# wangjiarui153/AIGV-Assessor

Measured on AMD Instinct MI355X. Metric: scored clips/sec (8-frame 448x448, InternVL2-8B stage-2 score eval), higher is better.
Workload: dtype bf16

## Files before the change

### aigv-assessor_amd/csrc/context.hip

```cpp
#include <cstdarg>
#include <cstdio>
#include <cstring>
#include <new>

#include "ctx.h"

using namespace aigv;

static thread_local std::string g_err;

int aigv::fail(aigv_ctx* c, int code, const char* fmt, ...) {
  char buf[512];
  va_list ap;
  va_start(ap, fmt);
  vsnprintf(buf, sizeof buf, fmt, ap);
  va_end(ap);
  if (c) c->err = buf;
  g_err = buf;
  return code;
}

static_assert(AIGV_MAX_KV_CAPACITY == AIGV_DECODE_MAX_CHUNKS * AIGV_DECODE_KEYS_PER_CHUNK, "the header's bound is the decode merge pass's");

static const char* kv_capacity_check(int kv_capacity) {
// ... 71 lines not shown
    if ((rc = dalloc(c, &c->l_t, T * k.llm_hidden))) break;
    if ((rc = dalloc(c, &c->l_qkv, T * c->qkv_out))) break;
    if ((rc = dalloc(c, &c->l_ao, T * k.llm_hidden))) break;
    if ((rc = dalloc(c, &c->l_ffn, T * k.llm_inter))) break;
    if ((rc = dalloc(c, &c->l_rows, (size_t)(k.max_out_rows + k.max_seqs + 64) * k.llm_hidden))) break;
    if ((rc = dalloc(c, &c->l_pos, T))) break;
    if ((rc = dalloc(c, &c->l_seq, T))) break;
    if ((rc = dalloc(c, &c->l_cu, (size_t)k.max_seqs + 1))) break;
    if ((rc = dalloc(c, &c->l_rowidx, (size_t)k.max_out_rows + k.max_seqs + 64))) break;
    if ((rc = dalloc(c, &c->l_rowidx2, (size_t)k.max_out_rows + k.max_seqs + 64))) break;
    if ((rc = dalloc(c, &c->l_kvlen, (size_t)k.max_seqs))) break;
    if ((rc = dalloc(c, &c->l_packed, (size_t)64))) break;
    if ((rc = dalloc(c, &c->l_trim, (size_t)64 * (2 * k.llm_hidden + k.llm_inter)))) break;
    if ((rc = dalloc(c, &c->l_trim_h, (size_t)(k.max_out_rows + k.max_seqs + 64) * k.llm_hidden))) break;
    if ((rc = dalloc(c, &c->l_neg1, (size_t)k.max_tokens))) break;
    c->rp_vit = RowPlan(); c->rp_llm = RowPlan(); c->cur_rp = nullptr;
    c->rp_vit.cap_halves = (int)(vr / 128) + 2 * k.vit_chunk + 2;
    c->rp_llm.cap_halves = (int)(T / 128) + 2 * k.max_seqs + 2;
    if ((rc = dalloc(c, &c->rp_vit.d_tab, (size_t)2 * c->rp_vit.cap_halves))) break;
    if ((rc = dalloc(c, &c->rp_llm.d_tab, (size_t)2 * c->rp_llm.cap_halves))) break;
    {
      const size_t widest = (size_t)std::max(std::max(std::max(2 * k.llm_inter, c->qkv_out), std::max(k.vit_inter, 3 * k.vit_hidden)), k.llm_hidden);
      const size_t rows = std::max((size_t)k.max_tokens, (size_t)k.vit_chunk * c->S);
      c->splitk_floats = std::min(SPLITK_MAX_FLOATS, (size_t)8 * rows * widest);
      void* p = nullptr;
      if (hipMalloc(&p, c->splitk_floats * sizeof(float)) != hipSuccess) { rc = fail(c, AIGV_ERR_ALLOC, "hipMalloc(split-K scratch) failed"); break; }
      c->ws_allocs.push_back(p);
      c->splitk_ws = (float*)p;
      if (hipMalloc(&p, c->splitk_floats * sizeof(float)) != hipSuccess) { rc = fail(c, AIGV_ERR_ALLOC, "hipMalloc(split-K scratch, InternViT) failed"); break; }
      c->ws_allocs.push_back(p);
      c->splitk_ws_vit = (float*)p;
    }
    if (hipMemset(c->l_neg1, 0xFF, (size_t)k.max_tokens * sizeof(int32_t)) != hipSuccess) { rc = fail(c, AIGV_ERR_HIP, "hipMemset failed"); break; }
    {
      int maxd = k.llm_hidden;
// ... 341 lines not shown
```

### aigv-assessor_amd/csrc/ctx.h

```cpp
#pragma once
#include <hip/hip_runtime.h>

#include <algorithm>
#include <string>
#include <unordered_map>
#include <vector>

#include "../../include/aigv_amd.h"
#include "kernels.h"

namespace aigv {

struct DevBuf {
  void* p = nullptr;
  size_t bytes = 0;
};

struct VitLayer {
  const bf16_t *ls1, *ls2, *qkv_w, *qkv_b, *qn, *kn, *proj_w, *proj_b, *fc1_w, *fc1_b, *fc2_w, *fc2_b, *n1w, *n1b, *n2w, *n2b;
};
struct LlmLayer {
  const bf16_t *wqkv, *wo, *w13, *w2, *an, *fn;
};

// ... 1 lines not shown
  uint8_t *wqkv = nullptr, *wo = nullptr, *w13 = nullptr, *w2 = nullptr;
  float *s_wqkv = nullptr, *s_wo = nullptr, *s_w13 = nullptr, *s_w2 = nullptr;
};

struct ProfRec {
  int cls;
  hipEvent_t a, b;
  double flops, bytes;
};

struct RowPlan {
  struct Tiny { int row0, stride_rows, count; };
  std::vector<Tiny> tiny;
  int rows = 0, body_halves = 0, tail_halves = 0, tail_rows = 0;
  int32_t* d_tab = nullptr;
  int cap_halves = 0;
};

}

struct aigv_ctx {
  aigv_config cfg{};
  int device = 0;
  std::string err;
  std::unordered_map<std::string, aigv::DevBuf> w;
  std::vector<void*> allocs;
  std::vector<void*> ws_allocs;
  bool ws_phase = false;
  bool finalized = false;
  int np = 0, S = 0, Kp = 0, grid = 0, ntok = 0, proj_in = 0, qkv_out = 0, head_dim = 0, vit_head_dim = 0, g = 0;
// ... 5 lines not shown
               *p_b1[2] = {nullptr, nullptr}, *p_w2[2] = {nullptr, nullptr}, *p_b2[2] = {nullptr, nullptr};
  ScoreHeadArgs score{};
  bf16_t *v_col = nullptr, *v_x = nullptr, *v_t = nullptr, *v_qkv = nullptr, *v_ao = nullptr, *v_h = nullptr;
  int32_t* v_cu = nullptr;
  bf16_t *p_t = nullptr, *p_mid = nullptr;
  bf16_t *l_h = nullptr, *l_t = nullptr, *l_qkv = nullptr, *l_ao = nullptr, *l_ffn = nullptr, *l_rows = nullptr;
  int32_t *l_pos = nullptr, *l_seq = nullptr, *l_cu = nullptr, *l_rowidx = nullptr, *l_rowidx2 = nullptr, *l_kvlen = nullptr;
  unsigned long long* l_packed = nullptr;
  int32_t* l_neg1 = nullptr;
  bool fp8_llm = false;
  bool llm_lin_dirty = false;
  std::vector<aigv::LlmLayerFp8> llm8;
  uint8_t* q8 = nullptr;
  float* q8_scale = nullptr;
  aigv::RowPlan rp_vit, rp_llm;
  const aigv::RowPlan* cur_rp = nullptr;
  bool trim_last_layer = true;
  int attn_round_scores = AIGV_ATTENTION_NUMERICS_DEFAULT;
  int tune[AIGV_TUNE_COUNT];
  aigv_ctx() { std::fill(tune, tune + AIGV_TUNE_COUNT, -1); }
  size_t splitk_floats = 0;
  float* splitk_ws = nullptr;
  float* splitk_ws_vit = nullptr;
  bool on_vit_front = false;
  bf16_t* l_trim = nullptr;
  bf16_t* l_trim_h = nullptr;
  bf16_t* l_score_ws = nullptr;
  bf16_t* l_lp = nullptr;
  int lp_ldo = 0;
  bf16_t *kc = nullptr, *vc = nullptr;
// ... 91 lines not shown

struct Tune {
  int v[AIGV_TUNE_COUNT];
  constexpr int operator[](int knob) const { return v[knob]; }
};
extern Tune g_tune;
inline int tune_knob(const aigv_ctx* c, int knob) { return (c && c->tune[knob] >= 0) ? c->tune[knob] : g_tune.v[knob]; }
inline int resolved_gemm_mode(const aigv_ctx* c) { return tune_knob(c, AIGV_TUNE_GEMM_MODE); }
inline Tune tune_of(const aigv_ctx* c) {
  Tune t;
  for (int k = 0; k < AIGV_TUNE_COUNT; ++k) t.v[k] = tune_knob(c, k);
  return t;
}

GemmArgs gemm_args(const bf16_t* A, int lda, const bf16_t* W, int ldw, bf16_t* C, int ldc, int M, int N, int K);
int build_row_plan(aigv_ctx* c, RowPlan& rp, const int32_t* cu, int n_seq, hipStream_t s);
int launch_one(aigv_ctx* c, const GemmArgs& a, int epi, bool use256, hipStream_t s);
int run_gemm(aigv_ctx* c, const GemmArgs& a, int epi, hipStream_t s);
int run_gemm_rows(aigv_ctx* c, const GemmArgs& a, int epi, const RowPlan& rp, hipStream_t s);
int run_gemm_full(aigv_ctx* c, const GemmArgs& a, int epi, hipStream_t s);
int run_llm_gemm(aigv_ctx* c, const GemmArgs& a, int epi, hipStream_t s);
int run_gemm_fp8(aigv_ctx* c, const bf16_t* A, int lda, int K, const uint8_t* W8, const float* w_scale, bf16_t* C, int ldc, int T, int N,
                 int epi, const bf16_t* resid, int ldr, hipStream_t s);
int run_skinny(aigv_ctx* c, const bf16_t* x, int ldx, int R, const bf16_t* W, int ldw, int N, int K, const bf16_t* bias,
               const bf16_t* resid, int ldr, bf16_t* out, int ldo, int epi, hipStream_t s, int p = 1);
constexpr size_t SPLITK_MAX_FLOATS = (size_t)64 << 20;
int splitk_scratch(aigv_ctx* c, size_t need_floats, float** out);
extern double g_rate256;

}
```

### aigv-assessor_amd/csrc/dispatch.hip

```cpp
#include <mutex>

#include "ctx.h"

namespace aigv {

static GemmArgs tuned(const aigv_ctx* c, const GemmArgs& a) {
  GemmArgs b = a;
  b.order_sel = tune_knob(c, AIGV_TUNE_GEMM256_ORDER); b.variant_sel = tune_knob(c, AIGV_TUNE_GEMM256_VARIANT);
  return b;
}
double g_rate256 = 1.46;
constexpr double KT128 = 0.95, FIX128 = 6.0, LONE128 = 0.70, FIX256 = 9.0, LAUNCH_GAP = 2.0;
static double kt256() { return 2.0 * KT128 / g_rate256; }

static double t256(long row_tiles, int N, int nk) {
  if (row_tiles <= 0) return 0;
  const long tiles = row_tiles * (N / 256);
  return (double)((tiles + 255) / 256) * (nk * kt256() + FIX256);
}
static double t128_blocks(long blocks, double nk_each) {
  const double rt = nk_each * KT128 + FIX128;
  const long full = blocks / 512, part = blocks % 512;
  return full * rt + (part == 0 ? 0.0 : part <= 256 ? LONE128 * rt : rt);
}
// ... 192 lines not shown
      const int sk = skinny_epi(epi);
      ProfScope ps(c, c ? c->gemm_cls : AIGV_PROF_GEMM, 2.0 * bot.M * (double)a.N * a.K, 2.0 * (double)a.N * a.K, s);
      hipError_t e = aigv_launch_skinny_gemm(bot.A, bot.lda, bot.M, bot.W, bot.ldw, bot.N, bot.K, bot.bias, bot.resid, bot.ldr,
                                            bot.C, bot.ldc, sk, s, bot.ls);
      if (e != hipSuccess) return fail(c, AIGV_ERR_HIP, "skinny remainder (M=%d N=%d K=%d): %s", bot.M, bot.N, bot.K, hipGetErrorString(e));
      return 0;
    }
    if (pl.last_slices > 1) return launch_splitk(c, bot, epi, pl.last_slices, false, s);
    return launch_one(c, bot, epi, false, s);
  }
  return 0;
}

constexpr int TINY_TAIL = 4;

int build_row_plan(aigv_ctx* c, RowPlan& rp, const int32_t* cu, int n_seq, hipStream_t s) {
  rp.tiny.clear();
  std::vector<int32_t> body, tail;
  bool uniform = true;
  for (int b = 1; b < n_seq; ++b) uniform = uniform && (cu[b + 1] - cu[b] == cu[1] - cu[0]);
  rp.tail_rows = 0;
  for (int b = 0; b < n_seq; ++b) {
    const int L = cu[b + 1] - cu[b], nb = L / 256, rem = L % 256, r0 = cu[b] + nb * 256;
    for (int j = 0; j < 2 * nb; ++j) { body.push_back(cu[b] + j * 128); body.push_back(128); }
    if (rem == 0) continue;
    if (rem <= TINY_TAIL) {
      if (!uniform) rp.tiny.push_back({r0, 1, rem});
      else if (b == 0)
        for (int j = 0; j < rem; ++j) rp.tiny.push_back({r0 + j, L, n_seq});
      continue;
    }
    tail.push_back(r0); tail.push_back(std::min(rem, 128));
    if (rem > 128) { tail.push_back(r0 + 128); tail.push_back(rem - 128); }
    rp.tail_rows += rem;
  }
  rp.body_halves = (int)body.size() / 2;
  rp.tail_halves = (int)tail.size() / 2;
  rp.rows = cu[n_seq];
  if (rp.body_halves + rp.tail_halves > rp.cap_halves)
    return fail(c, AIGV_ERR_STATE, "row plan: %d half tiles exceed the table's %d", rp.body_halves + rp.tail_halves, rp.cap_halves);
  body.insert(body.end(), tail.begin(), tail.end());
  if (!body.empty()) HIPCHK(c, aigv_launch_write_ints(body.data(), (int)body.size(), rp.d_tab, s));
  return 0;
}

static int tail_slices(int N, int K, int forced) {
  const int tn = N / 256, nk = K / 64;
  int best = 1;
  for (int S : {2, 4, 8})
    if (nk % S == 0 && nk / S >= 8 && 2 * tn * S <= 256) best = S;
  if (forced == 1 || (forced > 1 && nk % forced == 0 && nk / forced >= 4)) best = forced;
  return best;
}

static int launch_tab(aigv_ctx* c, const GemmArgs& a, int epi, const int32_t* tab, int halves, int rows, int S, hipStream_t s) {
  if (halves <= 0) return 0;
  GemmArgs b = tuned(c, a);
// ... 93 lines not shown
    if (!lone) TRY(launch_tab(c, a, epi, rp.d_tab, rp.body_halves, rp.body_halves * 128, 1, s));
  }
  if (tails_apart) {
    const size_t per_pair = (size_t)S * 256 * a.N;
    const size_t cap = c ? c->splitk_floats : SPLITK_MAX_FLOATS;
    const int max_halves = (int)std::min<size_t>(cap / per_pair, 4096) * 2;
    if (max_halves < 2) return fail(c, AIGV_ERR_STATE, "split-K scratch too small for one tail tile (N=%d, %d slices)", a.N, S);
    for (int h0 = 0; h0 < rp.tail_halves; h0 += max_halves) {
      const int nh = std::min(max_halves, rp.tail_halves - h0);
      TRY(launch_tab(c, a, epi, rp.d_tab + 2 * (rp.body_halves + h0), nh, nh * 128, S, s));
    }
  }
  return run_tiny_tails(c, a, epi, rp, s);
}

int run_gemm_full(aigv_ctx* c, const GemmArgs& a, int epi, hipStream_t s) {
  if (const char* m = aigv_gemm_check(a, epi)) return fail(c, AIGV_ERR_ARG, "%s (M=%d N=%d K=%d epi=%d)", m, a.M, a.N, a.K, epi);
  const int mode = resolved_gemm_mode(c);
  if (use_co(c, a, mode)) return launch_co(c, a, epi, s);
  if (mode == 1 || a.N < 256 || (a.N % 256 && epi == EPI_SWIGLU)) return launch_one(c, a, epi, false, s);
  if (a.N % 256) {
    TRY(launch_one(c, col_slice(a, 0, a.N - 128), epi, true, s));
    return launch_one(c, col_slice(a, a.N - 128, 128), epi, false, s);
  }
  return launch_one(c, a, epi, true, s);
}

int run_llm_gemm(aigv_ctx* c, const GemmArgs& a, int epi, hipStream_t s) {
  return c->cur_rp ? run_gemm_rows(c, a, epi, *c->cur_rp, s) : run_gemm(c, a, epi, s);
}
// ... 50 lines not shown
```

### aigv-assessor_amd/csrc/gemm256.hip

```cpp
#include <cstdlib>
#include <type_traits>

#include "common.h"
#include "kernels.h"

namespace {

constexpr int TM = 256, TN = 256, TK = 64;
constexpr int UNIT = 128 * 128;
constexpr int BUF = 4 * UNIT;
constexpr int STAGE_ROWP = 144;
constexpr int STAGE_BYTES = 16 * STAGE_ROWP;
constexpr int LDS_BYTES = 2 * BUF + 8 * STAGE_BYTES;
constexpr int GROUP_M256 = 4;
inline int row_tiles(const GemmArgs& a) { return a.row_tab ? (a.tab_halves + 1) / 2 : (a.M + TM - 1) / TM; }
}
static inline int tile_order(const GemmArgs& a, bool big_w, int nbm) { return a.order_sel > 0 ? a.order_sel - 1 : (big_w && nbm >= 32 ? 4 : 0); }
namespace {

#define RAW_BARRIER() asm volatile("s_barrier" ::: "memory")

#ifdef AIGV_GEMM_STAMP
constexpr int GSTAMP_REPL = 1024;
__device__ unsigned long long g_gemm_stamp[8][2][GSTAMP_REPL][8];
// ... 18 lines not shown
#endif
  (void)policy;
  *(u16x8*)dst = val;
}

template <int EPI, int VAR, bool FP8 = false, bool FUSE = false>
__global__ __launch_bounds__(512, 2) void gemm256_kernel(const GemmArgs p) {
  static_assert(!FP8 || ((VAR & 4) != 0 && EPI != EPI_PATCH), "the fp8 form uses the LDS-staged epilogue (or writes split-K slabs)");
  static_assert(!FUSE || (!FP8 && EPI != EPI_PARTIAL && EPI != EPI_PATCH), "the fused form: bf16, a body epilogue");
  extern __shared__ __attribute__((aligned(16))) char smem[];
  const int tid = threadIdx.x, lane = tid & 63;
  const int wave = __builtin_amdgcn_readfirstlane(tid >> 6);
  const int g = wave >> 2, wc = wave & 3;
  GSTAMP(gs_begin);

  const int nbm = p.row_tab ? (p.tab_halves + 1) / 2 : (p.M + TM - 1) / TM, nbn = p.N / TN;
  const int n_body = nbm * nbn;
  const bool is_slice = FUSE && (int)blockIdx.x >= n_body;
  const int nwg = is_slice ? ((p.fuse_tail_halves + 1) / 2) * nbn * p.k_slices : n_body;
  int wg;
  {
    const int bid = is_slice ? (int)blockIdx.x - n_body : (int)blockIdx.x, xcd = bid & 7, q = nwg >> 3, r = nwg & 7;
    wg = (xcd < r ? xcd * (q + 1) : r * (q + 1) + (xcd - r) * q) + (bid >> 3);
  }
  const bool partial = (EPI == EPI_PARTIAL) || is_slice;
  int slice_idx = (EPI == EPI_PARTIAL) ? (int)blockIdx.y : 0;
  int tm, tn;
  if (is_slice) {
    slice_idx = wg % p.k_slices;
    const int tile = wg / p.k_slices;
    tn = tile % nbn; tm = tile / nbn;
  } else if (p.order == 0) {
    const int per_group = GROUP_M256 * nbn;
    const int grp = wg / per_group, first_m = grp * GROUP_M256;
    const int gsz = min(nbm - first_m, GROUP_M256);
    const int in_g = wg - grp * per_group;
    tm = first_m + in_g % gsz; tn = in_g / gsz;
  } else {
    const int gn = p.order;
    const int per_group = gn * nbm;
    const int grp = wg / per_group, first_n = grp * gn;
    const int gsz = min(nbn - first_n, gn);
    const int in_g = wg - grp * per_group;
    tn = first_n + in_g % gsz; tm = in_g / gsz;
  }
  const int n0 = tn * TN;
  int hb, hv;
  if (p.row_tab) {
    const int h = 2 * tm + g;
    hb = 0; hv = 0;
    if (is_slice) {
      if (h < p.fuse_tail_halves) { hb = p.row_tab[2 * (p.tab_halves + h)]; hv = p.row_tab[2 * (p.tab_halves + h) + 1]; }
    } else if (h < p.tab_halves) { hb = p.row_tab[2 * h]; hv = p.row_tab[2 * h + 1]; }
  } else {
    hb = tm * TM + g * 128; hv = min(p.M - hb, 128);
    if (hv <= 0) { hb = p.M - 1; hv = 0; }
  }
  hb = __builtin_amdgcn_readfirstlane(hb);
  hv = __builtin_amdgcn_readfirstlane(hv);
  const int hend = hb + hv;
  auto relc = [&](int r) { return max(min(r, hv - 1), 0); };
// ... 458 lines not shown
            }
            u16x4 o;
#pragma unroll
            for (int e = 0; e < 4; ++e) o[e] = f2bf(v[e]);
            *(u16x4*)(p.C + orow * p.ldc + n) = o;
          }
      }
    }
  GSTAMP_FINISH();
}

template <int EPI, int VAR>
hipError_t launch256(const GemmArgs& a, hipStream_t s) {
  static LdsAttrOnce lds_attr;
  if (hipError_t e = lds_attr.ensure((const void*)gemm256_kernel<EPI, VAR>, LDS_BYTES); e != hipSuccess) return e;
  const int nbm = row_tiles(a), nbn = a.N / TN;
  GemmArgs b = a;
  b.order = tile_order(a, (size_t)a.N * (size_t)a.K >= ((size_t)32 << 20), nbm);
  hipLaunchKernelGGL((gemm256_kernel<EPI, VAR>), dim3(nbm * nbn), dim3(512), LDS_BYTES, s, b);
  return hipGetLastError();
}

template <int VAR>
hipError_t launch256v(const GemmArgs& a, int epi, hipStream_t s) {
  switch (epi) {
    case EPI_STORE: return launch256<EPI_STORE, VAR>(a, s);
    case EPI_GELU: return launch256<EPI_GELU, VAR>(a, s);
    case EPI_LS_RESID: return launch256<EPI_LS_RESID, VAR>(a, s);
    case EPI_RESID: return launch256<EPI_RESID, VAR>(a, s);
    case EPI_SWIGLU: return launch256<EPI_SWIGLU, VAR>(a, s);
    case EPI_PATCH: return launch256<EPI_PATCH, VAR>(a, s);
// ... 15 lines not shown
          unsigned long long t = 0;
          for (int r = 0; r < GSTAMP_REPL; ++r) t += host[e][c][r][i];
          out[(e * 2 + c) * 8 + i] = t;
        }
  }
  if (reset) {
    for (auto& a : host) for (auto& b : a) for (auto& c : b) for (auto& d : c) d = 0;
    if (hipMemcpyToSymbol(HIP_SYMBOL(g_gemm_stamp), host, sizeof host) != hipSuccess) return -2;
  }
  return 0;
}
#endif


bool aigv_gemm256_supported(const GemmArgs& a) { return a.N % TN == 0 && a.K % TK == 0 && a.M >= 1 && (!a.row_tab || a.tab_halves >= 1); }

template <int EPI>
hipError_t launch256_fp8(const GemmArgs& b, hipStream_t s) {
  static LdsAttrOnce lds_attr;
  if (hipError_t e = lds_attr.ensure((const void*)gemm256_kernel<EPI, 7, true>, LDS_BYTES); e != hipSuccess) return e;
  const int nbm = row_tiles(b), nbn = b.N / TN;
  GemmArgs c = b;
  c.order = tile_order(b, (size_t)b.N * (size_t)b.K * 2 >= ((size_t)64 << 20), nbm);
  hipLaunchKernelGGL((gemm256_kernel<EPI, 7, true>), dim3(nbm * nbn), dim3(512), LDS_BYTES, s, c);
  return hipGetLastError();
}

hipError_t aigv_launch_gemm256_fp8(const GemmArgs& a, int epi, hipStream_t s) {
  if (a.M < 1 || a.N % TN || a.K % 128 || (a.lda % 16) || (a.ldw % 16) || !a.row_scale || !a.col_scale || !a.A || !a.W || !a.C)
    return hipErrorInvalidValue;
  if ((epi == EPI_RESID || epi == EPI_LS_RESID) && (!a.resid || a.ldr % 8)) return hipErrorInvalidValue;
  if (epi == EPI_LS_RESID && !a.ls) return hipErrorInvalidValue;
  if (epi == EPI_SWIGLU && a.bias) return hipErrorInvalidValue;
  GemmArgs b = a;
  b.K = a.K / 2; b.lda = a.lda / 2; b.ldw = a.ldw / 2;
  switch (epi) {
    case EPI_STORE: return launch256_fp8<EPI_STORE>(b, s);
    case EPI_GELU: return launch256_fp8<EPI_GELU>(b, s);
    case EPI_LS_RESID: return launch256_fp8<EPI_LS_RESID>(b, s);
    case EPI_RESID: return launch256_fp8<EPI_RESID>(b, s);
    case EPI_SWIGLU: return launch256_fp8<EPI_SWIGLU>(b, s);
    default: return hipErrorInvalidValue;
  }
}

hipError_t aigv_launch_gemm256_fp8_partial(const GemmArgs& a, hipStream_t s) {
  if (a.M < 1 || a.N % TN || a.K % 128 || (a.lda % 16) || (a.ldw % 16) || !a.row_scale || !a.col_scale || !a.A || !a.W || !a.part || a.k_slices < 1 ||
      (a.K / 128) % a.k_slices)
    return hipErrorInvalidValue;
  static LdsAttrOnce lds_attr;
  if (hipError_t e = lds_attr.ensure((const void*)gemm256_kernel<EPI_PARTIAL, 7, true>, LDS_BYTES); e != hipSuccess) return e;
  GemmArgs b = a;
  b.K = a.K / 2; b.lda = a.lda / 2; b.ldw = a.ldw / 2;
  const int nbm = row_tiles(a), nbn = a.N / TN;
  hipLaunchKernelGGL((gemm256_kernel<EPI_PARTIAL, 7, true>), dim3(nbm * nbn, a.k_slices), dim3(512), LDS_BYTES, s, b);
  return hipGetLastError();
}

hipError_t aigv_launch_gemm256_partial(const GemmArgs& a, hipStream_t s) {
  if (!aigv_gemm256_supported(a) || a.k_slices < 1 || (a.K / TK) % a.k_slices || !a.part) return hipErrorInvalidValue;
  static LdsAttrOnce lds_attr;
  if (hipError_t e = lds_attr.ensure((const void*)gemm256_kernel<EPI_PARTIAL, 7>, LDS_BYTES); e != hipSuccess) return e;
  const int nbm = row_tiles(a), nbn = a.N / TN;
  hipLaunchKernelGGL((gemm256_kernel<EPI_PARTIAL, 7>), dim3(nbm * nbn, a.k_slices), dim3(512), LDS_BYTES, s, a);
  return hipGetLastError();
}

template <int EPI>
static hipError_t launch256_fused(const GemmArgs& a, hipStream_t s) {
  static LdsAttrOnce lds_attr;
  if (hipError_t e = lds_attr.ensure((const void*)gemm256_kernel<EPI, 7, false, true>, LDS_BYTES); e != hipSuccess) return e;
  const int nbm = (a.tab_halves + 1) / 2, nbn = a.N / TN;
  GemmArgs b = a;
  b.order = tile_order(a, (size_t)a.N * (size_t)a.K >= ((size_t)32 << 20), nbm);
  b.fuse_body_wg = nbm * nbn;
  const int grid = nbm * nbn + ((a.fuse_tail_halves + 1) / 2) * nbn * a.k_slices;
  hipLaunchKernelGGL((gemm256_kernel<EPI, 7, false, true>), dim3(grid), dim3(512), LDS_BYTES, s, b);
  return hipGetLastError();
}

hipError_t aigv_launch_gemm256_fused(const GemmArgs& a, int epi, hipStream_t s) {
  if (!aigv_gemm256_supported(a) || !a.row_tab || (a.tab_halves & 1) || a.fuse_tail_halves < 1 || a.k_slices < 2 || (a.K / TK) % a.k_slices || !a.part)
    return hipErrorInvalidValue;
  switch (epi) {
    case EPI_STORE: return launch256_fused<EPI_STORE>(a, s);
    case EPI_GELU: return launch256_fused<EPI_GELU>(a, s);
    case EPI_LS_RESID: return launch256_fused<EPI_LS_RESID>(a, s);
    case EPI_RESID: return launch256_fused<EPI_RESID>(a, s);
    case EPI_SWIGLU: return launch256_fused<EPI_SWIGLU>(a, s);
  }
  return hipErrorInvalidValue;
}

hipError_t aigv_launch_gemm256(const GemmArgs& a, int epi, hipStream_t s) {
  switch (a.variant_sel > 0 ? a.variant_sel - 1 : 1) {
    case 0: return launch256v<0>(a, epi, s);
    case 3: return launch256v<3>(a, epi, s);
    default: return launch256v<7>(a, epi, s);
  }
}
```

### aigv-assessor_amd/csrc/kernels.h

```cpp
#pragma once
#include <hip/hip_runtime.h>
#include <stdint.h>

typedef uint16_t bf16_t;

enum GemmEpilogue {
  EPI_STORE = 0,
  EPI_GELU = 1,
  EPI_LS_RESID = 2,
  EPI_RESID = 3,
  EPI_SWIGLU = 4,
  EPI_PATCH = 5,
  EPI_COUNT = 6,
  EPI_PARTIAL = 6
};

struct GemmArgs {
  const bf16_t* A; int lda;
  const bf16_t* W; int ldw;
  bf16_t* C; int ldc;
  const bf16_t* bias;
  const bf16_t* ls;
  const bf16_t* resid; int ldr;
  const bf16_t* pos;
  int M, N, K;
  int np;
  float* part;
  int k_slices;
  const float* row_scale;
  const float* col_scale;
  const int32_t* row_tab; int tab_halves;
  int fuse_tail_halves, fuse_body_wg;
  int order_sel, variant_sel;
  int order;
};

const char* aigv_gemm_check(const GemmArgs& a, int epi);
hipError_t aigv_launch_gemm(const GemmArgs& a, int epi, hipStream_t s);
hipError_t aigv_launch_gemm_splitk(const GemmArgs& a, int epi, int k_slices, float* ws, hipStream_t s, bool tile256 = false);
hipError_t aigv_launch_gemm256_partial(const GemmArgs& a, hipStream_t s);
hipError_t aigv_launch_gemm256_fp8(const GemmArgs& a, int epi, hipStream_t s);
hipError_t aigv_launch_gemm256_fp8_partial(const GemmArgs& a, hipStream_t s);
hipError_t aigv_launch_gemm_splitk_fp8(const GemmArgs& a, int epi, int k_slices, float* ws, hipStream_t s);
hipError_t aigv_launch_rmsnorm_quant_fp8(const bf16_t* x, int ldx, const bf16_t* w, uint8_t* q, int ldq, float* scale, int rows, int H, float eps,
                                         hipStream_t s);
hipError_t aigv_launch_quant_fp8_rows(const bf16_t* x, int ldx, int rows, int K, uint8_t* q, int ldq, float* scale, hipStream_t s);
bool aigv_gemm256_supported(const GemmArgs& a);
hipError_t aigv_launch_gemm256_fused(const GemmArgs& a, int epi, hipStream_t s);
// ... 122 lines not shown
```

### aigv-assessor_amd/csrc/passes.hip

```cpp
#include <cmath>

#include "ctx.h"

using namespace aigv;

extern "C" {

static int vit_norm(aigv_ctx* c, const bf16_t* x, const bf16_t* w, const bf16_t* b, bf16_t* y, int rows, hipStream_t s) {
  const aigv_config& k = c->cfg;
  if (k.vit_norm_rms) HIPCHK(c, aigv_launch_rmsnorm(x, k.vit_hidden, w, y, k.vit_hidden, rows, k.vit_hidden, k.vit_eps, nullptr, s));
  else HIPCHK(c, aigv_launch_layernorm(x, k.vit_hidden, w, b, y, k.vit_hidden, rows, k.vit_hidden, k.vit_eps, s));
  return 0;
}

int aigv_vit_forward(aigv_ctx* c, const void* frames, int n_frames, void* out_tokens, void* stream) {
  if (!c || !frames || !out_tokens) return fail(c, AIGV_ERR_ARG, "aigv_vit_forward: null argument");
  if (!c->finalized) return fail(c, AIGV_ERR_STATE, "aigv_vit_forward: call aigv_finalize_weights first");
  const aigv_config& k = c->cfg;
  if (n_frames <= 0 || n_frames > k.max_frames) return fail(c, AIGV_ERR_ARG, "n_frames %d outside 1..%d", n_frames, k.max_frames);
  HIPCHK(c, hipSetDevice(c->device));
  hipStream_t s = (hipStream_t)stream;
  GemmClassScope gcls(c, AIGV_PROF_GEMM_VIT);
  SplitkVitScope svs(c);
  const int Hv = k.vit_hidden, Iv = k.vit_inter;
// ... 138 lines not shown
  HIPCHK(c, aigv_launch_rmsnorm(hidden, H, c->final_norm, c->l_rows, H, n, H, k.rms_eps, compact ? nullptr : c->l_rowidx, s));
  for (int b0 = 0; b0 < nS; b0 += 64) {
    ScoreHeadArgs a = c->score;
    a.x = c->l_rows + (size_t)b0 * H; a.ldx = H; a.B = std::min(64, nS - b0); a.score = score + b0;
    HIPCHK(c, aigv_launch_score_head(a, c->l_score_ws, s));
  }
  for (int r0 = 0; r0 < R; r0 += 64) {
    const int rr = std::min(64, R - r0);
    ProfScope ps(c, AIGV_PROF_SKINNY, 2.0 * rr * (double)k.vocab * H, 2.0 * (double)k.vocab * H, s);
    HIPCHK(c, aigv_launch_lm_head_argmax(c->l_rows + (size_t)(nS + r0) * H, rr, H, c->lm_head, k.vocab, c->l_packed,
                                         argmax + r0, nullptr, s));
  }
  return 0;
}

static int llm_layer_qkv(aigv_ctx* c, int li, int T, hipStream_t s) {
  const aigv_config& k = c->cfg;
  const LlmLayer& L = c->llm[li];
  const int H = k.llm_hidden, D = c->head_dim, g = c->g, nkv = k.llm_kv_heads;
  if (c->fp8_llm) {
    HIPCHK(c, aigv_launch_rmsnorm_quant_fp8(c->l_h, H, L.an, c->q8, H, c->q8_scale, T, H, k.rms_eps, s));
    TRY(run_gemm_fp8(c, nullptr, H, H, c->llm8[li].wqkv, c->llm8[li].s_wqkv, c->l_qkv, c->qkv_out, T, c->qkv_out, EPI_STORE, nullptr, 0, s));
  } else {
    HIPCHK(c, aigv_launch_rmsnorm(c->l_h, H, L.an, c->l_t, H, T, H, k.rms_eps, nullptr, s));
    TRY(run_llm_gemm(c, gemm_args(c->l_t, H, L.wqkv, H, c->l_qkv, c->qkv_out, T, c->qkv_out, H), EPI_STORE, s));
  }
  HIPCHK(c, aigv_launch_rope(c->l_qkv, c->qkv_out, c->l_pos, c->rope_cos, c->rope_sin, T, 1, g + 2, nkv, D, s, g));
  return 0;
}

static int llm_layer_post(aigv_ctx* c, int li, int T, hipStream_t s) {
  const aigv_config& k = c->cfg;
  const LlmLayer& L = c->llm[li];
  const int H = k.llm_hidden, I = k.llm_inter;
  if (c->fp8_llm && li != k.llm_layers - 1) {
    const LlmLayerFp8& Q = c->llm8[li];
    TRY(run_gemm_fp8(c, c->l_ao, H, H, Q.wo, Q.s_wo, c->l_h, H, T, H, EPI_RESID, c->l_h, H, s));
    HIPCHK(c, aigv_launch_rmsnorm_quant_fp8(c->l_h, H, L.fn, c->q8, H, c->q8_scale, T, H, k.rms_eps, s));
    TRY(run_gemm_fp8(c, nullptr, H, H, Q.w13, Q.s_w13, c->l_ffn, I, T, 2 * I, EPI_SWIGLU, nullptr, 0, s));
    TRY(run_gemm_fp8(c, c->l_ffn, I, I, Q.w2, Q.s_w2, c->l_h, H, T, H, EPI_RESID, c->l_h, H, s));
// ... 82 lines not shown
    std::vector<int> per_clip(B, 0), clip_of(c->h_rowidx.size());
    for (size_t i = 0; i < c->h_rowidx.size(); ++i) {
      int b = 0;
      while (cu[b + 1] <= c->h_rowidx[i]) ++b;
      clip_of[i] = b;
      ++per_clip[b];
      q_tail = std::max(q_tail, cu[b + 1] - c->h_rowidx[i]);
    }
    for (size_t i = 0; i < c->h_rowidx.size(); ++i)
      if (per_clip[clip_of[i]] <= TRIM_ROWS) small_rows.push_back(c->h_rowidx[i]);
  }
  const bool trim_ok = c->trim_last_layer && n_out > 0 && H % 128 == 0 && I % 128 == 0;
  const bool trim = trim_ok && (int)small_rows.size() == n_out;
  const bool mixed = trim_ok && !trim && !small_rows.empty();
  if (mixed) HIPCHK(c, aigv_launch_write_ints(small_rows.data(), (int)small_rows.size(), c->l_rowidx2, s));
  double attn_flops = 0;
  for (int b = 0; b < B; ++b) { const double L = cu[b + 1] - cu[b]; attn_flops += 4.0 * (L * (L + 1) / 2) * D * k.llm_heads; }
  const size_t kv_layer = (size_t)k.max_seqs * nkv * k.kv_capacity * D;
  for (int li = 0; li < k.llm_layers; ++li) {
    const LlmLayer& L = c->llm[li];
    TRY(llm_layer_qkv(c, li, T, s));
    if (keep_kv)
      HIPCHK(c, aigv_launch_kv_store(c->l_qkv, c->qkv_out, c->l_seq, c->l_pos, c->kc + li * kv_layer, c->vc + li * kv_layer, T,
                                     nkv, g, D, k.kv_capacity, s));
    if (n_out == 0 && c->trim_last_layer && li == k.llm_layers - 1) break;
    {
      AttnArgs a = llm_attn_args(c, B);
      a.k = c->l_qkv + (size_t)g * D; a.v = c->l_qkv + (size_t)(g + 1) * D;
      a.ldk = a.ldv = c->qkv_out; a.kv_head_stride = (g + 2) * D;
      a.max_len = max_len;
      const bool last_trim = trim && li == k.llm_layers - 1;
      a.q_tail = last_trim ? q_tail : 0;
      if (const char* m = aigv_attn_check(a, D)) return fail(c, AIGV_ERR_ARG, "%s", m);
      ProfScope ps(c, AIGV_PROF_ATTN_LLM, last_trim ? 0.0 : attn_flops, 2.0 * T * ((double)c->qkv_out + H), s);
      HIPCHK(c, aigv_launch_attention(a, D, s));
    }
// ... 389 lines not shown
```

### aigv-assessor_amd/csrc/tune.hip

```cpp
#include "ctx.h"

using namespace aigv;

namespace {

constexpr bool in_waves(int v) { return v == 0 || v == 4 || v == 8; }
constexpr bool in_forms(int v) { return v == 0 || v == 1 || v == 2 || v == 4; }
constexpr bool in_forms_packed(int v) { return in_forms(v) || (v >= 1000 && v < 1000 + 4096); }
constexpr bool in_kmax(int v) { return v >= 0 && v <= 65536 && v % 64 == 0; }

struct Knob {
  int def;
  int hi;
  bool (*in_set)(int);
  bool process_default;
};
constexpr Knob KNOBS[AIGV_TUNE_COUNT] = {
    {0, 4, nullptr, false},
    {0, 15, nullptr, false},
    {0, 7, nullptr, false},
    {0, 0, in_waves, false},
    {0, 0, in_forms_packed, false},
    {0, 2, nullptr, false},
    {0, 0, in_kmax, true},
    {0, 16, nullptr, true},
    {0, 1, nullptr, true},
    {1, 1, nullptr, false},
    {1, 1, nullptr, false},
    {0, 0, in_forms, false},
    {0, 2, nullptr, true},
    {1, 4, nullptr, true},
};
static_assert(AIGV_TUNE_GEMM_MODE == 0 && AIGV_TUNE_CO_KMAX == 6 && AIGV_TUNE_LONE_BODY == 13 && AIGV_TUNE_COUNT == 14, "KNOBS follows the enum's order");

constexpr Tune library_defaults() {
  Tune t{};
  for (int k = 0; k < AIGV_TUNE_COUNT; ++k) t.v[k] = KNOBS[k].def;
  return t;
}

bool known(int knob) { return knob >= 0 && knob < AIGV_TUNE_COUNT; }
bool valid(int knob, int value) { return KNOBS[knob].in_set ? KNOBS[knob].in_set(value) : value >= 0 && value <= KNOBS[knob].hi; }

}

Tune aigv::g_tune = library_defaults();

extern "C" {
// ... 105 lines not shown
```

### aigv-assessor_amd/modeling.py

```python
from __future__ import annotations

import ctypes as C
import os
from typing import Dict, List, Optional

import torch
import torch.nn as nn
import torch.nn.functional as F

from . import native, synth
from .config import InternVLChatConfig
from .conversation import get_conv_template


def rope_tables(head_dim: int, theta: float, n_pos: int, max_pos: int = 32768, scaling: Optional[dict] = None,
                seq_len: Optional[int] = None):
    base = float(theta)
    if scaling is not None and scaling.get("type") == "dynamic" and seq_len is not None and seq_len > max_pos:
        f = float(scaling["factor"])
        base = base * ((f * seq_len / max_pos) - (f - 1)) ** (head_dim / (head_dim - 2))
    inv_freq = 1.0 / (base ** (torch.arange(0, head_dim, 2).float() / head_dim))
    t = torch.arange(n_pos).to(inv_freq.dtype)
    if scaling is not None and scaling.get("type") == "linear":
        t = t / float(scaling["factor"])
# ... 1444 lines not shown
    def set_attention_numerics(self, mode: str = "fp32"):
        self._drop_graphs()
        if mode not in ("reference", "fp32"):
            raise ValueError("attention numerics must be 'reference' or 'fp32'")
        self._attn_numerics = 1 if mode == "reference" else 0
        lib, ctx = self._native()
        native.check(lib.aigv_set_attention_numerics(ctx, self._attn_numerics), ctx)

    def set_gemm_mode(self, mode: int = -1):
        self._drop_graphs()
        self._gemm_mode = int(mode)
        lib, ctx = self._native()
        native.check(lib.aigv_set_gemm_mode(ctx, int(mode)), ctx)

    TUNE_KNOBS = {"gemm_mode": 0, "gemm256_order": 1, "gemm256_variant": 2, "attn_waves": 3, "skinny_p": 4, "body_tile": 5, "co_kmax": 6,
                  "tail_slices": 7, "attn_lead_key": 8, "decode_fused": 9, "decode_fp8": 10, "skinny_p8": 11, "fuse_tails": 12, "lone_body": 13}

    def tune(self, knob: str, value: int = -1):
        self._drop_graphs()
        lib, ctx = self._native()
        native.check(lib.aigv_ctx_tune(ctx, self.TUNE_KNOBS[knob], int(value)), ctx)

    def capture_forward(self, **forward_kwargs):
        pv = forward_kwargs.get("pixel_values")
        if torch.is_tensor(pv) and forward_kwargs.get("motion_feature") is None and forward_kwargs.get("input_ids") is not None:
            self._prepare_motion_branch(pv, int(forward_kwargs["input_ids"].shape[0]))
        torch.cuda.synchronize(self.device)
        graph = torch.cuda.CUDAGraph()
        self._capture_keep = []
        try:
            with native.capturing(), torch.cuda.graph(graph, capture_error_mode="relaxed"):
# ... 33 lines not shown
```

### include/aigv_amd.h

```cpp
#ifndef AIGV_AMD_H
#define AIGV_AMD_H

#include <stdint.h>

#ifdef __cplusplus
extern "C" {
#endif

#define AIGV_ABI_VERSION 3

#define AIGV_MAX_CANDIDATES 64
#define AIGV_MAX_TOPK 16

#define AIGV_MAX_KV_CAPACITY 262144

typedef struct aigv_ctx aigv_ctx;

enum aigv_status {
  AIGV_OK = 0,
  AIGV_ERR_ARG = -1,
  AIGV_ERR_HIP = -2,
  AIGV_ERR_STATE = -3,
  AIGV_ERR_ALLOC = -4
};
// ... 146 lines not shown
enum aigv_tune_knob {
  AIGV_TUNE_GEMM_MODE = 0,
  AIGV_TUNE_GEMM256_ORDER = 1,
  AIGV_TUNE_GEMM256_VARIANT = 2,
  AIGV_TUNE_ATTN_WAVES = 3,
  AIGV_TUNE_SKINNY_P = 4,
  AIGV_TUNE_BODY_TILE = 5,
  AIGV_TUNE_CO_KMAX = 6,
  AIGV_TUNE_TAIL_SLICES = 7,
  AIGV_TUNE_ATTN_LEAD_KEY = 8,
  AIGV_TUNE_DECODE_FUSED = 9,
  AIGV_TUNE_DECODE_FP8 = 10,
  AIGV_TUNE_SKINNY_P8 = 11,
  AIGV_TUNE_FUSE_TAILS = 12,
  AIGV_TUNE_LONE_BODY = 13,
  AIGV_TUNE_COUNT = 14
};
int aigv_ctx_tune(aigv_ctx* ctx, int knob, int value);
int aigv_tune_gemm(int mode, double rate256);
int aigv_tune_co_gemm(int kmax);
int aigv_tune_default(int knob, int value);
int aigv_plan_gemm(int M, int N, int K, int epi, int* plan, double* est_us);
int aigv_tune_attention(int waves);
int aigv_tune_skinny(int p);

enum aigv_prof_class { AIGV_PROF_GEMM = 0, AIGV_PROF_ATTN_VIT = 1, AIGV_PROF_ATTN_LLM = 2, AIGV_PROF_SKINNY = 3,
                       AIGV_PROF_GEMM_FP8 = 4, AIGV_PROF_GEMM_VIT = 5, AIGV_PROF_COUNT = 6 };
int aigv_prof_enable(aigv_ctx* ctx, int on);
int aigv_prof_read(aigv_ctx* ctx, int cls, int64_t* launches, double* total_ms, double* flops, double* bytes);

typedef struct aigv_slowfast aigv_slowfast;
// ... 41 lines not shown
```

Measured before the change: 35.03.

## Compute only K/V columns for leading row tiles in last LLM layer QKV

```diff
diff --git a/aigv-assessor_amd/csrc/context.hip b/aigv-assessor_amd/csrc/context.hip
--- a/aigv-assessor_amd/csrc/context.hip
+++ b/aigv-assessor_amd/csrc/context.hip
@@ -109,11 +109,13 @@
     if ((rc = dalloc(c, &c->l_trim, (size_t)64 * (2 * k.llm_hidden + k.llm_inter)))) break;
     if ((rc = dalloc(c, &c->l_trim_h, (size_t)(k.max_out_rows + k.max_seqs + 64) * k.llm_hidden))) break;
     if ((rc = dalloc(c, &c->l_neg1, (size_t)k.max_tokens))) break;
-    c->rp_vit = RowPlan(); c->rp_llm = RowPlan(); c->cur_rp = nullptr;
+    c->rp_vit = RowPlan(); c->rp_llm = RowPlan(); c->rp_llm_last = RowPlan(); c->cur_rp = nullptr;
     c->rp_vit.cap_halves = (int)(vr / 128) + 2 * k.vit_chunk + 2;
     c->rp_llm.cap_halves = (int)(T / 128) + 2 * k.max_seqs + 2;
     if ((rc = dalloc(c, &c->rp_vit.d_tab, (size_t)2 * c->rp_vit.cap_halves))) break;
     if ((rc = dalloc(c, &c->rp_llm.d_tab, (size_t)2 * c->rp_llm.cap_halves))) break;
+    c->rp_llm_last.cap_halves = c->rp_llm.cap_halves;
+    if ((rc = dalloc(c, &c->rp_llm_last.d_tab, (size_t)2 * c->rp_llm_last.cap_halves))) break;
     {
       const size_t widest = (size_t)std::max(std::max(std::max(2 * k.llm_inter, c->qkv_out), std::max(k.vit_inter, 3 * k.vit_hidden)), k.llm_hidden);
       const size_t rows = std::max((size_t)k.max_tokens, (size_t)k.vit_chunk * c->S);
diff --git a/aigv-assessor_amd/csrc/ctx.h b/aigv-assessor_amd/csrc/ctx.h
--- a/aigv-assessor_amd/csrc/ctx.h
+++ b/aigv-assessor_amd/csrc/ctx.h
@@ -39,6 +39,7 @@
   std::vector<Tiny> tiny;
   int rows = 0, body_halves = 0, tail_halves = 0, tail_rows = 0;
   int32_t* d_tab = nullptr;
+  int front_halves = 0;
   int cap_halves = 0;
 };
 
@@ -74,6 +75,7 @@
   uint8_t* q8 = nullptr;
   float* q8_scale = nullptr;
   aigv::RowPlan rp_vit, rp_llm;
+  aigv::RowPlan rp_llm_last;
   const aigv::RowPlan* cur_rp = nullptr;
   bool trim_last_layer = true;
   int attn_round_scores = AIGV_ATTENTION_NUMERICS_DEFAULT;
@@ -195,12 +197,14 @@
 }
 
 GemmArgs gemm_args(const bf16_t* A, int lda, const bf16_t* W, int ldw, bf16_t* C, int ldc, int M, int N, int K);
-int build_row_plan(aigv_ctx* c, RowPlan& rp, const int32_t* cu, int n_seq, hipStream_t s);
+int build_row_plan(aigv_ctx* c, RowPlan& rp, const int32_t* cu, int n_seq, hipStream_t s, const int* front = nullptr);
 int launch_one(aigv_ctx* c, const GemmArgs& a, int epi, bool use256, hipStream_t s);
 int run_gemm(aigv_ctx* c, const GemmArgs& a, int epi, hipStream_t s);
 int run_gemm_rows(aigv_ctx* c, const GemmArgs& a, int epi, const RowPlan& rp, hipStream_t s);
 int run_gemm_full(aigv_ctx* c, const GemmArgs& a, int epi, hipStream_t s);
 int run_llm_gemm(aigv_ctx* c, const GemmArgs& a, int epi, hipStream_t s);
+int run_gemm_rows_kv_front(aigv_ctx* c, const GemmArgs& a, int epi, const RowPlan& rp, int col_stride, int col_off, hipStream_t s);
+bool kv_front_runnable(const aigv_ctx* c, const GemmArgs& a);
 int run_gemm_fp8(aigv_ctx* c, const bf16_t* A, int lda, int K, const uint8_t* W8, const float* w_scale, bf16_t* C, int ldc, int T, int N,
                  int epi, const bf16_t* resid, int ldr, hipStream_t s);
 int run_skinny(aigv_ctx* c, const bf16_t* x, int ldx, int R, const bf16_t* W, int ldw, int N, int K, const bf16_t* bias,
diff --git a/aigv-assessor_amd/csrc/dispatch.hip b/aigv-assessor_amd/csrc/dispatch.hip
--- a/aigv-assessor_amd/csrc/dispatch.hip
+++ b/aigv-assessor_amd/csrc/dispatch.hip
@@ -230,15 +230,16 @@
 
 constexpr int TINY_TAIL = 4;
 
-int build_row_plan(aigv_ctx* c, RowPlan& rp, const int32_t* cu, int n_seq, hipStream_t s) {
+int build_row_plan(aigv_ctx* c, RowPlan& rp, const int32_t* cu, int n_seq, hipStream_t s, const int* front) {
   rp.tiny.clear();
-  std::vector<int32_t> body, tail;
+  std::vector<int32_t> body, tail, lead;
   bool uniform = true;
   for (int b = 1; b < n_seq; ++b) uniform = uniform && (cu[b + 1] - cu[b] == cu[1] - cu[0]);
   rp.tail_rows = 0;
   for (int b = 0; b < n_seq; ++b) {
     const int L = cu[b + 1] - cu[b], nb = L / 256, rem = L % 256, r0 = cu[b] + nb * 256;
-    for (int j = 0; j < 2 * nb; ++j) { body.push_back(cu[b] + j * 128); body.push_back(128); }
+    const int nf = front ? std::min(std::max(front[b], 0), nb) : 0;
+    for (int j = 0; j < 2 * nb; ++j) { std::vector<int32_t>& v = j < 2 * nf ? lead : body; v.push_back(cu[b] + j * 128); v.push_back(128); }
     if (rem == 0) continue;
     if (rem <= TINY_TAIL) {
       if (!uniform) rp.tiny.push_back({r0, 1, rem});
@@ -250,13 +251,15 @@
     if (rem > 128) { tail.push_back(r0 + 128); tail.push_back(rem - 128); }
     rp.tail_rows += rem;
   }
+  rp.front_halves = (int)lead.size() / 2;
   rp.body_halves = (int)body.size() / 2;
   rp.tail_halves = (int)tail.size() / 2;
   rp.rows = cu[n_seq];
-  if (rp.body_halves + rp.tail_halves > rp.cap_halves)
-    return fail(c, AIGV_ERR_STATE, "row plan: %d half tiles exceed the table's %d", rp.body_halves + rp.tail_halves, rp.cap_halves);
-  body.insert(body.end(), tail.begin(), tail.end());
-  if (!body.empty()) HIPCHK(c, aigv_launch_write_ints(body.data(), (int)body.size(), rp.d_tab, s));
+  if (rp.front_halves + rp.body_halves + rp.tail_halves > rp.cap_halves)
+    return fail(c, AIGV_ERR_STATE, "row plan: %d half tiles exceed the table's %d", rp.front_halves + rp.body_halves + rp.tail_halves, rp.cap_halves);
+  lead.insert(lead.end(), body.begin(), body.end());
+  lead.insert(lead.end(), tail.begin(), tail.end());
+  if (!lead.empty()) HIPCHK(c, aigv_launch_write_ints(lead.data(), (int)lead.size(), rp.d_tab, s));
   return 0;
 }
 
@@ -380,6 +383,26 @@
   return run_tiny_tails(c, a, epi, rp, s);
 }
 
+bool kv_front_runnable(const aigv_ctx* c, const GemmArgs& a) {
+  const int mode = resolved_gemm_mode(c);
+  return mode == 0 && !use_co(c, a, mode) && a.N >= 256 && a.N % 256 == 0 && aigv_gemm256_supported(a) && tune_knob(c, AIGV_TUNE_BODY_TILE) != 2 &&
+         tune_knob(c, AIGV_TUNE_LONE_BODY) == 1;
+}
+
+int run_gemm_rows_kv_front(aigv_ctx* c, const GemmArgs& a, int epi, const RowPlan& rp, int col_stride, int col_off, hipStream_t s) {
+  if (a.M != rp.rows) return fail(c, AIGV_ERR_STATE, "row plan covers %d rows, the GEMM has %d", rp.rows, a.M);
+  if (rp.front_halves > 0) {
+    GemmArgs b = tuned(c, a);
+    b.row_tab = rp.d_tab; b.tab_halves = rp.front_halves; b.col_stride = col_stride; b.col_off = col_off;
+    const double rows = rp.front_halves * 128.0, n = (double)a.N / col_stride;
+    ProfScope ps(c, c ? c->gemm_cls : AIGV_PROF_GEMM, 2.0 * rows * n * a.K, 2.0 * (rows * a.K + n * a.K + rows * n), s);
+    HIPCHK(c, aigv_launch_gemm256(b, epi, s));
+  }
+  RowPlan rest = rp;
+  rest.d_tab = rp.d_tab + 2 * rp.front_halves; rest.front_halves = 0;
+  return run_gemm_rows(c, a, epi, rest, s);
+}
+
 int run_gemm_full(aigv_ctx* c, const GemmArgs& a, int epi, hipStream_t s) {
   if (const char* m = aigv_gemm_check(a, epi)) return fail(c, AIGV_ERR_ARG, "%s (M=%d N=%d K=%d epi=%d)", m, a.M, a.N, a.K, epi);
   const int mode = resolved_gemm_mode(c);
diff --git a/aigv-assessor_amd/csrc/gemm256.hip b/aigv-assessor_amd/csrc/gemm256.hip
--- a/aigv-assessor_amd/csrc/gemm256.hip
+++ b/aigv-assessor_amd/csrc/gemm256.hip
@@ -56,7 +56,8 @@
   const int g = wave >> 2, wc = wave & 3;
   GSTAMP(gs_begin);
 
-  const int nbm = p.row_tab ? (p.tab_halves + 1) / 2 : (p.M + TM - 1) / TM, nbn = p.N / TN;
+  const int cstride = max(p.col_stride, 1);
+  const int nbm = p.row_tab ? (p.tab_halves + 1) / 2 : (p.M + TM - 1) / TM, nbn = p.N / TN / cstride;
   const int n_body = nbm * nbn;
   const bool is_slice = FUSE && (int)blockIdx.x >= n_body;
   const int nwg = is_slice ? ((p.fuse_tail_halves + 1) / 2) * nbn * p.k_slices : n_body;
@@ -86,7 +87,7 @@
     const int in_g = wg - grp * per_group;
     tn = first_n + in_g % gsz; tm = in_g / gsz;
   }
-  const int n0 = tn * TN;
+  const int n0 = (tn * cstride + p.col_off) * TN;
   int hb, hv;
   if (p.row_tab) {
     const int h = 2 * tm + g;
@@ -575,7 +576,7 @@
 hipError_t launch256(const GemmArgs& a, hipStream_t s) {
   static LdsAttrOnce lds_attr;
   if (hipError_t e = lds_attr.ensure((const void*)gemm256_kernel<EPI, VAR>, LDS_BYTES); e != hipSuccess) return e;
-  const int nbm = row_tiles(a), nbn = a.N / TN;
+  const int nbm = row_tiles(a), nbn = a.N / TN / (a.col_stride > 1 ? a.col_stride : 1);
   GemmArgs b = a;
   b.order = tile_order(a, (size_t)a.N * (size_t)a.K >= ((size_t)32 << 20), nbm);
   hipLaunchKernelGGL((gemm256_kernel<EPI, VAR>), dim3(nbm * nbn), dim3(512), LDS_BYTES, s, b);
@@ -621,6 +622,7 @@
 
 
 bool aigv_gemm256_supported(const GemmArgs& a) { return a.N % TN == 0 && a.K % TK == 0 && a.M >= 1 && (!a.row_tab || a.tab_halves >= 1); }
+static bool all_columns(const GemmArgs& a) { return a.col_stride <= 1 && a.col_off == 0; }
 
 template <int EPI>
 hipError_t launch256_fp8(const GemmArgs& b, hipStream_t s) {
@@ -634,7 +636,7 @@
 }
 
 hipError_t aigv_launch_gemm256_fp8(const GemmArgs& a, int epi, hipStream_t s) {
-  if (a.M < 1 || a.N % TN || a.K % 128 || (a.lda % 16) || (a.ldw % 16) || !a.row_scale || !a.col_scale || !a.A || !a.W || !a.C)
+  if (a.M < 1 || a.N % TN || a.K % 128 || (a.lda % 16) || (a.ldw % 16) || !a.row_scale || !a.col_scale || !a.A || !a.W || !a.C || !all_columns(a))
     return hipErrorInvalidValue;
   if ((epi == EPI_RESID || epi == EPI_LS_RESID) && (!a.resid || a.ldr % 8)) return hipErrorInvalidValue;
   if (epi == EPI_LS_RESID && !a.ls) return hipErrorInvalidValue;
@@ -653,7 +655,7 @@
 
 hipError_t aigv_launch_gemm256_fp8_partial(const GemmArgs& a, hipStream_t s) {
   if (a.M < 1 || a.N % TN || a.K % 128 || (a.lda % 16) || (a.ldw % 16) || !a.row_scale || !a.col_scale || !a.A || !a.W || !a.part || a.k_slices < 1 ||
-      (a.K / 128) % a.k_slices)
+      (a.K / 128) % a.k_slices || !all_columns(a))
     return hipErrorInvalidValue;
   static LdsAttrOnce lds_attr;
   if (hipError_t e = lds_attr.ensure((const void*)gemm256_kernel<EPI_PARTIAL, 7, true>, LDS_BYTES); e != hipSuccess) return e;
@@ -665,7 +667,7 @@
 }
 
 hipError_t aigv_launch_gemm256_partial(const GemmArgs& a, hipStream_t s) {
-  if (!aigv_gemm256_supported(a) || a.k_slices < 1 || (a.K / TK) % a.k_slices || !a.part) return hipErrorInvalidValue;
+  if (!aigv_gemm256_supported(a) || a.k_slices < 1 || (a.K / TK) % a.k_slices || !a.part || !all_columns(a)) return hipErrorInvalidValue;
   static LdsAttrOnce lds_attr;
   if (hipError_t e = lds_attr.ensure((const void*)gemm256_kernel<EPI_PARTIAL, 7>, LDS_BYTES); e != hipSuccess) return e;
   const int nbm = row_tiles(a), nbn = a.N / TN;
@@ -687,7 +689,7 @@
 }
 
 hipError_t aigv_launch_gemm256_fused(const GemmArgs& a, int epi, hipStream_t s) {
-  if (!aigv_gemm256_supported(a) || !a.row_tab || (a.tab_halves & 1) || a.fuse_tail_halves < 1 || a.k_slices < 2 || (a.K / TK) % a.k_slices || !a.part)
+  if (!aigv_gemm256_supported(a) || !a.row_tab || (a.tab_halves & 1) || a.fuse_tail_halves < 1 || a.k_slices < 2 || (a.K / TK) % a.k_slices || !a.part || !all_columns(a))
     return hipErrorInvalidValue;
   switch (epi) {
     case EPI_STORE: return launch256_fused<EPI_STORE>(a, s);
@@ -700,6 +702,7 @@
 }
 
 hipError_t aigv_launch_gemm256(const GemmArgs& a, int epi, hipStream_t s) {
+  if (a.col_stride > 1 ? (a.N / TN) % a.col_stride != 0 || a.col_off < 0 || a.col_off >= a.col_stride : !all_columns(a)) return hipErrorInvalidValue;
   switch (a.variant_sel > 0 ? a.variant_sel - 1 : 1) {
     case 0: return launch256v<0>(a, epi, s);
     case 3: return launch256v<3>(a, epi, s);
diff --git a/aigv-assessor_amd/csrc/kernels.h b/aigv-assessor_amd/csrc/kernels.h
--- a/aigv-assessor_amd/csrc/kernels.h
+++ b/aigv-assessor_amd/csrc/kernels.h
@@ -32,6 +32,7 @@
   const int32_t* row_tab; int tab_halves;
   int fuse_tail_halves, fuse_body_wg;
   int order_sel, variant_sel;
+  int col_stride, col_off;
   int order;
 };
 
diff --git a/aigv-assessor_amd/csrc/passes.hip b/aigv-assessor_amd/csrc/passes.hip
--- a/aigv-assessor_amd/csrc/passes.hip
+++ b/aigv-assessor_amd/csrc/passes.hip
@@ -176,7 +176,7 @@
   return 0;
 }
 
-static int llm_layer_qkv(aigv_ctx* c, int li, int T, hipStream_t s) {
+static int llm_layer_qkv(aigv_ctx* c, int li, int T, hipStream_t s, bool kv_front = false) {
   const aigv_config& k = c->cfg;
   const LlmLayer& L = c->llm[li];
   const int H = k.llm_hidden, D = c->head_dim, g = c->g, nkv = k.llm_kv_heads;
@@ -185,7 +185,9 @@
     TRY(run_gemm_fp8(c, nullptr, H, H, c->llm8[li].wqkv, c->llm8[li].s_wqkv, c->l_qkv, c->qkv_out, T, c->qkv_out, EPI_STORE, nullptr, 0, s));
   } else {
     HIPCHK(c, aigv_launch_rmsnorm(c->l_h, H, L.an, c->l_t, H, T, H, k.rms_eps, nullptr, s));
-    TRY(run_llm_gemm(c, gemm_args(c->l_t, H, L.wqkv, H, c->l_qkv, c->qkv_out, T, c->qkv_out, H), EPI_STORE, s));
+    const GemmArgs a = gemm_args(c->l_t, H, L.wqkv, H, c->l_qkv, c->qkv_out, T, c->qkv_out, H);
+    if (kv_front) TRY(run_gemm_rows_kv_front(c, a, EPI_STORE, c->rp_llm_last, (g + 2) / 2, g / 2, s));
+    else TRY(run_llm_gemm(c, a, EPI_STORE, s));
   }
   HIPCHK(c, aigv_launch_rope(c->l_qkv, c->qkv_out, c->l_pos, c->rope_cos, c->rope_sin, T, 1, g + 2, nkv, D, s, g));
   return 0;
@@ -298,12 +300,22 @@
   const bool trim = trim_ok && (int)small_rows.size() == n_out;
   const bool mixed = trim_ok && !trim && !small_rows.empty();
   if (mixed) HIPCHK(c, aigv_launch_write_ints(small_rows.data(), (int)small_rows.size(), c->l_rowidx2, s));
+  bool kv_front = false;
+  if (trim && !c->fp8_llm && tune_knob(c, AIGV_TUNE_LAST_KV_TILES) == 1 && D == 128 && g % 2 == 0 &&
+      kv_front_runnable(c, gemm_args(c->l_t, H, c->llm[k.llm_layers - 1].wqkv, H, c->l_qkv, c->qkv_out, T, c->qkv_out, H))) {
+    std::vector<int> front(B);
+    for (int b = 0; b < B; ++b) {
+      front[b] = std::max(0, (cu[b + 1] - cu[b] - q_tail) / 256);
+      kv_front = kv_front || front[b] > 0;
+    }
+    if (kv_front) TRY(build_row_plan(c, c->rp_llm_last, cu, B, s, front.data()));
+  }
   double attn_flops = 0;
   for (int b = 0; b < B; ++b) { const double L = cu[b + 1] - cu[b]; attn_flops += 4.0 * (L * (L + 1) / 2) * D * k.llm_heads; }
   const size_t kv_layer = (size_t)k.max_seqs * nkv * k.kv_capacity * D;
   for (int li = 0; li < k.llm_layers; ++li) {
     const LlmLayer& L = c->llm[li];
-    TRY(llm_layer_qkv(c, li, T, s));
+    TRY(llm_layer_qkv(c, li, T, s, kv_front && li == k.llm_layers - 1));
     if (keep_kv)
       HIPCHK(c, aigv_launch_kv_store(c->l_qkv, c->qkv_out, c->l_seq, c->l_pos, c->kc + li * kv_layer, c->vc + li * kv_layer, T,
                                      nkv, g, D, k.kv_capacity, s));
diff --git a/aigv-assessor_amd/csrc/tune.hip b/aigv-assessor_amd/csrc/tune.hip
--- a/aigv-assessor_amd/csrc/tune.hip
+++ b/aigv-assessor_amd/csrc/tune.hip
@@ -30,8 +30,9 @@
     {0, 0, in_forms, false},
     {0, 2, nullptr, true},
     {1, 4, nullptr, true},
+    {1, 1, nullptr, true},
 };
-static_assert(AIGV_TUNE_GEMM_MODE == 0 && AIGV_TUNE_CO_KMAX == 6 && AIGV_TUNE_LONE_BODY == 13 && AIGV_TUNE_COUNT == 14, "KNOBS follows the enum's order");
+static_assert(AIGV_TUNE_GEMM_MODE == 0 && AIGV_TUNE_CO_KMAX == 6 && AIGV_TUNE_LONE_BODY == 13 && AIGV_TUNE_LAST_KV_TILES == 14 && AIGV_TUNE_COUNT == 15, "KNOBS follows the enum's order");
 
 constexpr Tune library_defaults() {
   Tune t{};
diff --git a/aigv-assessor_amd/modeling.py b/aigv-assessor_amd/modeling.py
--- a/aigv-assessor_amd/modeling.py
+++ b/aigv-assessor_amd/modeling.py
@@ -1482,7 +1482,8 @@
         native.check(lib.aigv_set_gemm_mode(ctx, int(mode)), ctx)
 
     TUNE_KNOBS = {"gemm_mode": 0, "gemm256_order": 1, "gemm256_variant": 2, "attn_waves": 3, "skinny_p": 4, "body_tile": 5, "co_kmax": 6,
-                  "tail_slices": 7, "attn_lead_key": 8, "decode_fused": 9, "decode_fp8": 10, "skinny_p8": 11, "fuse_tails": 12, "lone_body": 13}
+                  "tail_slices": 7, "attn_lead_key": 8, "decode_fused": 9, "decode_fp8": 10, "skinny_p8": 11, "fuse_tails": 12, "lone_body": 13,
+                  "last_kv_tiles": 14}
 
     def tune(self, knob: str, value: int = -1):
         self._drop_graphs()
diff --git a/include/aigv_amd.h b/include/aigv_amd.h
--- a/include/aigv_amd.h
+++ b/include/aigv_amd.h
@@ -184,7 +184,8 @@
   AIGV_TUNE_SKINNY_P8 = 11,
   AIGV_TUNE_FUSE_TAILS = 12,
   AIGV_TUNE_LONE_BODY = 13,
-  AIGV_TUNE_COUNT = 14
+  AIGV_TUNE_LAST_KV_TILES = 14,
+  AIGV_TUNE_COUNT = 15
 };
 int aigv_ctx_tune(aigv_ctx* ctx, int knob, int value);
 int aigv_tune_gemm(int mode, double rate256);
```

After: 35.08 (median of 6 runs). Within noise of the previous version (+0.1%).
